# taiyaki-go/motioncheck_ccm_slam

Hardware: AMD Instinct MI355X
Metric: ORB extract+match Mfeatures/s and GBA iter/s (2k KF, 200k pts) @1/2/4/8 GPU (higher is better)
Workload: dtype u8; 1 GPU; configs[1]: 256 synthetic 752x480 frames per GPU, 8-level pyramid, 1000 features, FAST+quadtree+rBRIEF, then 1000x1000 brute-force Hamming on the 255 consecutive pairs; frames_per_gpu=256

## Files before the change

### include/ccm_hot.h

```cpp
#ifndef CCM_HOT_H
#define CCM_HOT_H

#include <stddef.h>
#include <stdint.h>

#ifdef __cplusplus
extern "C" {
#endif

#define CCM_ABI_VERSION 3

enum {
    CCM_OK = 0,
    CCM_E_ARG = -1,
    CCM_E_DEVICE = -2,
    CCM_E_NOMEM = -3,
    CCM_E_CAPACITY = -4,
    CCM_E_NUMERIC = -5,
    CCM_E_COMM = -6,
    CCM_E_STATE = -7
};

typedef struct ccm_ctx ccm_ctx;

// ... 16 lines not shown

typedef struct {
    int   nfeatures;
    float scale_factor;
    int   nlevels;
    int   ini_th_fast;
    int   min_th_fast;
} ccm_orb_params;

#define CCM_MAX_LEVELS 16

typedef struct {
    float x, y;
    float size;
    float angle;
    float response;
    int32_t octave;
    int32_t class_id;
} ccm_keypoint;

int ccm_orb_tables(const ccm_orb_params*, float* scale, float* inv_scale, float* sigma2,
                   float* inv_sigma2, int32_t* features_per_level, int32_t* umax);
int ccm_orb_level_sizes(const ccm_orb_params*, int w, int h, int32_t* level_w, int32_t* level_h);

int ccm_orb_extract(ccm_ctx*, const ccm_orb_params*, const uint8_t* img, int w, int h, int stride,
                    size_t image_stride, int n_images, ccm_keypoint* kps, uint8_t* desc,
                    int32_t* counts, int max_per_image);

int ccm_orb_extract_dev(ccm_ctx*, const ccm_orb_params*, const uint8_t* img_dev, int w, int h,
                        int stride, size_t image_stride, int n_images, int max_per_image);
int ccm_orb_fetch(ccm_ctx*, ccm_keypoint* kps, uint8_t* desc, int32_t* counts);
int ccm_orb_result_dev(ccm_ctx*, const uint8_t** desc_dev, const int32_t** counts_dev,
                       int* max_per_image);

int ccm_orb_debug_level(ccm_ctx*, int image, int level, uint8_t* out, int out_stride);
int ccm_orb_debug_candidates(ccm_ctx*, int image, int level, int32_t* xy, int32_t* score, int max);

int ccm_descriptor_distance(const uint8_t* a, const uint8_t* b);

int ccm_hamming_match(ccm_ctx*, const uint8_t* q, int nq, const uint8_t* t, int nt, int n_pairs,
                      const int32_t* nq_n, const int32_t* nt_n,
                      int32_t* best_idx, int32_t* best_dist, int32_t* second_dist);
int ccm_hamming_match_dev(ccm_ctx*, const uint8_t* q_dev, int nq, size_t q_pair_stride,
                          const uint8_t* t_dev, int nt, size_t t_pair_stride, int n_pairs,
                          const int32_t* nq_n_dev, const int32_t* nt_n_dev,
                          int32_t* best_idx_dev, int32_t* best_dist_dev, int32_t* second_dist_dev);
// ... 248 lines not shown
```

### motioncheck_ccm_slam_amd/_lib.py

```python
from __future__ import annotations

import ctypes as C
import os

import numpy as np

_HERE = os.path.dirname(os.path.abspath(__file__))
LIB_PATH = os.environ.get("CCM_HOT_LIB") or os.path.join(_HERE, "libccm_hot.so")

CCM_OK = 0
ERRORS = {-1: "CCM_E_ARG", -2: "CCM_E_DEVICE", -3: "CCM_E_NOMEM", -4: "CCM_E_CAPACITY",
          -5: "CCM_E_NUMERIC", -6: "CCM_E_COMM", -7: "CCM_E_STATE"}
COMM_ID_BYTES = 128

KP_DTYPE = np.dtype([("x", "f4"), ("y", "f4"), ("size", "f4"), ("angle", "f4"), ("response", "f4"),
                     ("octave", "i4"), ("class_id", "i4")])

SYMBOLS = [
    "ccm_abi_version", "ccm_create", "ccm_destroy", "ccm_last_error", "ccm_sync", "ccm_stream",
    "ccm_host_register", "ccm_host_unregister", "ccm_profile_enable", "ccm_profile_read",
    "ccm_orb_tables", "ccm_orb_level_sizes", "ccm_orb_extract", "ccm_orb_extract_dev", "ccm_orb_fetch",
    "ccm_orb_result_dev", "ccm_orb_debug_level", "ccm_orb_debug_candidates",
    "ccm_descriptor_distance", "ccm_hamming_match", "ccm_hamming_match_dev", "ccm_ratio_test", "ccm_match_bow",
    "ccm_window_candidates", "ccm_search_by_projection", "ccm_search_by_projection_frame", "ccm_search_for_initialization", "ccm_fuse_select", "ccm_fuse_select_batch", "ccm_search_by_sim3", "ccm_search_by_projection_sim3", "ccm_search_by_projection_sim3_batch",
    "ccm_search_for_triangulation", "ccm_voc_create", "ccm_voc_destroy", "ccm_voc_words", "ccm_voc_transform", "ccm_voc_transform_dev",
    "ccm_bow_vector", "ccm_bow_score_l1", "ccm_distinctive_descriptors", "ccm_optimize_sim3", "ccm_optimize_essential_graph", "ccm_correct_map_points",
    "ccm_ba_solve", "ccm_ba_landmark_cuts", "ccm_pose_optimize", "ccm_comm_unique_id", "ccm_comm_init", "ccm_comm_attach", "ccm_comm_destroy",
    "ccm_pose_from_mat4f", "ccm_pose_to_mat4f",
    "ccm_frame_create", "ccm_frame_from_extract", "ccm_frame_destroy", "ccm_frame_size", "ccm_frame_set_map_points",
    "ccm_frame_get_map_points", "ccm_frame_debug_grid", "ccm_frame_search_by_projection", "ccm_frame_search_by_projection_frame",
    "ccm_frame_pose_optimize",
    "ccm_sim3_ransac_iterations", "ccm_sim3_solver_create", "ccm_sim3_solver_destroy", "ccm_sim3_solver_count", "ccm_sim3_solver_iterate",
    "ccm_sim3_solver_find", "ccm_sim3_solver_estimate", "ccm_sim3_solver_state", "ccm_sim3_solver_hypotheses",
]


class CcmError(RuntimeError):
    def __init__(self, code, text=""):
        super().__init__("%s (%d): %s" % (ERRORS.get(code, "CCM_E_?"), code, text))
        self.code = code


class OrbParams(C.Structure):
    _fields_ = [("nfeatures", C.c_int), ("scale_factor", C.c_float), ("nlevels", C.c_int),
# ... 68 lines not shown
    if not os.path.exists(LIB_PATH):
        raise ImportError("%s not found: build it with `make -C motioncheck_ccm_slam_amd/csrc` "
                          "(or __graft_entry__.build()); there is no CPU fallback" % LIB_PATH)
    lib = C.CDLL(LIB_PATH)
    if lib.ccm_abi_version() != ABI_VERSION:
        raise ImportError("%s has ABI version %d, this package mirrors version %d of include/ccm_hot.h: rebuild it"
                          % (LIB_PATH, lib.ccm_abi_version(), ABI_VERSION))
    lib.ccm_create.restype = C.c_void_p
    lib.ccm_create.argtypes = [C.c_int, C.c_int]
    lib.ccm_destroy.argtypes = [C.c_void_p]
    lib.ccm_destroy.restype = None
    lib.ccm_last_error.restype = C.c_char_p
    lib.ccm_last_error.argtypes = [C.c_void_p]
    lib.ccm_sync.argtypes = [C.c_void_p]
    lib.ccm_stream.restype = C.c_void_p
    lib.ccm_stream.argtypes = [C.c_void_p]
    vp = C.c_void_p
    lib.ccm_host_register.argtypes = [vp, vp, C.c_size_t]
    lib.ccm_host_unregister.argtypes = [vp, vp]
    lib.ccm_profile_enable.argtypes = [vp, C.c_int]
    lib.ccm_profile_read.argtypes = [vp, vp, vp]
    lib.ccm_orb_tables.argtypes = [C.POINTER(OrbParams)] + [vp] * 6
    lib.ccm_orb_level_sizes.argtypes = [C.POINTER(OrbParams), C.c_int, C.c_int, vp, vp]
    lib.ccm_orb_extract.argtypes = [vp, C.POINTER(OrbParams), vp, C.c_int, C.c_int, C.c_int, C.c_size_t, C.c_int,
                                    vp, vp, vp, C.c_int]
    lib.ccm_orb_extract_dev.argtypes = [vp, C.POINTER(OrbParams), vp, C.c_int, C.c_int, C.c_int, C.c_size_t,
                                        C.c_int, C.c_int]
    lib.ccm_orb_fetch.argtypes = [vp, vp, vp, vp]
    lib.ccm_orb_result_dev.argtypes = [vp, C.POINTER(vp), C.POINTER(vp), C.POINTER(C.c_int)]
    lib.ccm_orb_debug_level.argtypes = [vp, C.c_int, C.c_int, vp, C.c_int]
    lib.ccm_orb_debug_candidates.argtypes = [vp, C.c_int, C.c_int, vp, vp, C.c_int]
    lib.ccm_descriptor_distance.argtypes = [vp, vp]
    lib.ccm_hamming_match.argtypes = [vp, vp, C.c_int, vp, C.c_int, C.c_int, vp, vp, vp, vp, vp]
    lib.ccm_hamming_match_dev.argtypes = [vp, vp, C.c_int, C.c_size_t, vp, C.c_int, C.c_size_t, C.c_int,
                                          vp, vp, vp, vp, vp]
    lib.ccm_ratio_test.argtypes = [C.c_int, C.c_int, C.c_float, C.c_int, C.c_int]
    lib.ccm_match_bow.argtypes = [vp, C.POINTER(BowOptions), vp, vp, vp, vp, C.c_int, vp, vp, vp, vp, C.c_int, vp]
    lib.ccm_window_candidates.argtypes = [vp, C.POINTER(FrameGrid), C.c_int, vp, vp, vp, vp, vp, vp, C.c_int, vp, vp, vp]
    lib.ccm_search_by_projection.argtypes = [vp, C.POINTER(FrameGrid), vp, C.c_int, vp, vp, vp, vp, vp, vp, vp, vp, C.c_float, C.c_float, vp]
    lib.ccm_search_by_projection_frame.argtypes = [vp, C.POINTER(FrameGrid), vp, vp, C.c_int, vp, vp, vp, vp, vp, vp, vp, vp, C.c_float, C.c_int, C.c_int, vp]
    lib.ccm_search_for_initialization.argtypes = [vp, C.c_int, vp, vp, vp, C.POINTER(FrameGrid), vp, vp, C.c_int, C.c_float, C.c_int, vp]
    lib.ccm_fuse_select.argtypes = [vp, C.POINTER(FrameGrid), vp, vp, C.c_int, vp, vp, vp, vp, vp, C.c_float, C.c_int, C.c_int, vp, vp]
    lib.ccm_fuse_select_batch.argtypes = [vp, C.c_int, vp, vp, vp, vp, vp, vp, vp, vp, vp, C.c_float, C.c_int, C.c_int, vp, vp]
    lib.ccm_search_by_sim3.argtypes = [vp, C.POINTER(FrameGrid), vp, C.POINTER(FrameGrid), vp] + [vp] * 10 + [C.c_float, vp]
    lib.ccm_search_by_projection_sim3.argtypes = [vp, C.POINTER(FrameGrid), vp, C.c_int] + [vp] * 7 + [C.c_float, vp]
    lib.ccm_search_by_projection_sim3_batch.argtypes = [vp, C.c_int, vp, vp, vp] + [vp] * 7 + [C.c_float, vp, vp]
# ... 111 lines not shown
```

### motioncheck_ccm_slam_amd/csrc/orb_host.cpp

```cpp
#include "ccm_internal.h"
#include "orb_types.h"
#include <cmath>
#include <cfloat>
#include <algorithm>

extern "C" hipError_t orb_upload_pattern();
size_t orb_octree_lds_bytes(int list_cap);
void orb_launch_resize(hipStream_t, const OrbGeom&, int level, int dw, int dh, int nframes);
void orb_launch_score(hipStream_t, const OrbGeom&, int ntiles, int nframes);
void orb_launch_nms(hipStream_t, const OrbGeom&, const OrbCell*, int ncells, int nframes, unsigned* slots, int* cell_count);
void orb_launch_fast_cells(hipStream_t, const OrbGeom&, const OrbCell*, const OrbBand*, int nbands, int nframes, size_t lds_bytes,
                           int surv_cap, unsigned* slots, int* cell_count);
size_t orb_fast_cells_lds(int pitch, int bh, int surv_cap);
void orb_launch_octree(hipStream_t, const OrbGeom&, const OrbCell*, int nlevels, int nframes, int list_cap,
                       const unsigned* slots, const int* cell_count, unsigned* keysA, unsigned* keysB,
                       unsigned* out, int* out_count, int* status);
void orb_launch_orient_desc(hipStream_t, const OrbGeom&, int out_per_frame, int nframes, const unsigned* sel,
                            const int* sel_count, ccm_keypoint* kps, uint8_t* desc, int* counts, int max_per_image,
                            int* status);

namespace {

inline int cv_round(float v) { return (int)lrintf(v); }
inline int cv_round(double v) { return (int)lrint(v); }

struct OrbTables {
    float scale[ORB_MAX_LEVELS], inv_scale[ORB_MAX_LEVELS], sigma2[ORB_MAX_LEVELS], inv_sigma2[ORB_MAX_LEVELS];
    int nfeat[ORB_MAX_LEVELS];
    int umax[16];
};

// ... 29 lines not shown
        t->umax[v] = v0;
        ++v0;
    }
    return CCM_OK;
}

void linear_tables(int ssize, int dsize, std::vector<int>& ofs, std::vector<short>& ab)
{
    ofs.resize(dsize); ab.resize(2 * (size_t)dsize);
    const double inv_scale = (double)dsize / ssize;
    const double scale = 1. / inv_scale;
    for (int d = 0; d < dsize; d++) {
        float fx = (float)((d + 0.5) * scale - 0.5);
        int sx = (int)std::floor(fx);
        fx -= sx;
        if (sx < 0) { sx = 0; fx = 0.f; }
        if (sx >= ssize - 1) { sx = ssize - 1; fx = 0.f; }
        ofs[d] = sx;
        ab[2 * d] = (short)cv_round((1.f - fx) * 2048.f);
        ab[2 * d + 1] = (short)cv_round(fx * 2048.f);
    }
}

}

struct OrbState {
    ccm_orb_params par{}; int w = 0, h = 0, nframes = 0, max_per_image = 0;
    bool valid = false, pattern_up = false;
    OrbTables tab{};
    OrbGeom geom{};
    std::vector<OrbCell> cells;
    std::vector<OrbBand> bands; size_t band_lds = 0; bool fused = true; int surv_cap = 1024; hipStream_t copy_stream = nullptr; hipEvent_t copy_done = nullptr;
    hipStream_t down_stream = nullptr; hipEvent_t chunk_done = nullptr;
    DevBuf geom_dev, cells_dev, tables_dev, bands_dev;
    DevBuf pyr, smap, slots, cell_count, keysA, keysB, sel, sel_count, status;
    DevBuf img0;
    DevBuf kps, desc, counts;
    size_t pyr_off[ORB_MAX_LEVELS]{}, smap_off[ORB_MAX_LEVELS]{};
    const uint8_t* last_img = nullptr; int last_stride = 0; size_t last_image_stride = 0;
    bool have_result = false;
};

void orb_state_free(OrbState* s)
{
    if (!s) return;
    if (s->copy_done) (void)hipEventDestroy(s->copy_done);
    if (s->chunk_done) (void)hipEventDestroy(s->chunk_done);
    delete s;
}

static inline size_t align_up(size_t v, size_t a) { return (v + a - 1) / a * a; }

static int orb_prepare(ccm_ctx* c, const ccm_orb_params* p, int w, int h, int nframes, int max_per_image)
{
    if (!c->orb) c->orb = new OrbState();
    OrbState& S = *c->orb;
    const bool same = S.valid && std::memcmp(&S.par, p, sizeof *p) == 0 && S.w == w && S.h == h &&
                      S.nframes == nframes && S.max_per_image == max_per_image;
    if (same) return CCM_OK;
    S.valid = false; S.have_result = false;
    int rc = make_tables(p, &S.tab);
    if (rc) return ccm_fail(c, rc, "bad ORB parameters");
    if (p->ini_th_fast < 0 || p->ini_th_fast > 255 || p->min_th_fast < 0 || p->min_th_fast > 255)
        return ccm_fail(c, CCM_E_ARG, "FAST thresholds must be in [0,255]");
    OrbGeom& G = S.geom;
    std::memset(&G, 0, sizeof G);
    G.nlevels = p->nlevels; G.ini_th = p->ini_th_fast; G.min_th = p->min_th_fast;
    for (int i = 0; i < 16; i++) G.umax[i] = S.tab.umax[i];
    S.cells.clear();
    std::vector<int> tab_i; std::vector<short> tab_s;
    struct TabOff { size_t xofs, yofs, xab, yab; } toff[ORB_MAX_LEVELS]{};
    size_t pyr_bytes = 0, smap_bytes = 0;
    int slot_acc = 0, key_acc = 0, out_acc = 0, tile_acc = 0, max_quota = 0;
    for (int l = 0; l < p->nlevels; l++) {
        OrbLevel& L = G.lv[l];
        L.w = cv_round((float)w * S.tab.inv_scale[l]);
        L.h = cv_round((float)h * S.tab.inv_scale[l]);
        if (L.w < 2 * ORB_EDGE + 8 || L.h < 2 * ORB_EDGE + 8 || L.w > 4096 + 2 * ORB_BORDER || L.h > 4096 + 2 * ORB_BORDER)
            return ccm_fail(c, CCM_E_ARG, "level %d is %dx%d: unsupported image size", l, L.w, L.h);
        L.scale = S.tab.scale[l];
        L.kp_size = (float)(int)(31 * S.tab.scale[l]);
        L.quota = S.tab.nfeat[l];
        max_quota = std::max(max_quota, L.quota);
        L.spitch = (int)align_up(L.w, 64);
        L.splane = (long long)L.spitch * L.h;
        S.smap_off[l] = smap_bytes; smap_bytes += align_up((size_t)L.splane * nframes, 256);
        if (l > 0) {
            L.pitch = (int)align_up(L.w, 64);
            L.plane = (long long)L.pitch * L.h;
            S.pyr_off[l] = pyr_bytes; pyr_bytes += align_up((size_t)L.plane * nframes, 256);
            std::vector<int> xo, yo; std::vector<short> xa, ya;
            linear_tables(G.lv[l - 1].w, L.w, xo, xa);
            linear_tables(G.lv[l - 1].h, L.h, yo, ya);
            toff[l].xofs = tab_i.size(); tab_i.insert(tab_i.end(), xo.begin(), xo.end());
            toff[l].yofs = tab_i.size(); tab_i.insert(tab_i.end(), yo.begin(), yo.end());
            toff[l].xab = tab_s.size(); tab_s.insert(tab_s.end(), xa.begin(), xa.end());
            toff[l].yab = tab_s.size(); tab_s.insert(tab_s.end(), ya.begin(), ya.end());
        }
        const int minBX = ORB_BORDER, minBY = ORB_BORDER, maxBX = L.w - ORB_EDGE + 3, maxBY = L.h - ORB_EDGE + 3;
        const float width = (float)(maxBX - minBX), height = (float)(maxBY - minBY);
        const int nCols = (int)(width / 30.f), nRows = (int)(height / 30.f);
        L.bw = maxBX - minBX; L.bh = maxBY - minBY;
        L.cell_first = (int)S.cells.size();
        int key_cap = 0;
        if (nCols >= 1 && nRows >= 1) {
            const int wCell = (int)std::ceil(width / nCols), hCell = (int)std::ceil(height / nRows);
            for (int i = 0; i < nRows; i++) {
                const float iniY = (float)(minBY + i * hCell);
                float maxY = iniY + hCell + 6;
                if (iniY >= maxBY - 3) continue;
                if (maxY > maxBY) maxY = (float)maxBY;
                for (int j = 0; j < nCols; j++) {
                    const float iniX = (float)(minBX + j * wCell);
                    float maxX = iniX + wCell + 6;
                    if (iniX >= maxBX - 6) continue;
                    if (maxX > maxBX) maxX = (float)maxBX;
                    OrbCell cell{};
                    cell.level = (short)l; cell.x0 = (short)iniX; cell.y0 = (short)iniY;
                    cell.cw = (short)((int)maxX - (int)iniX); cell.ch = (short)((int)maxY - (int)iniY);
                    if (cell.cw > 65 || cell.ch > 65)
                        return ccm_fail(c, CCM_E_ARG, "FAST cell %dx%d exceeds the kernel tile", cell.cw, cell.ch);
                    const int rw = std::max(cell.cw - 6, 0), rh = std::max(cell.ch - 6, 0);
                    cell.slot_cap = ((rw + 1) / 2) * ((rh + 1) / 2);
                    cell.slot_first = slot_acc;
                    slot_acc += cell.slot_cap; key_cap += cell.slot_cap;
                    S.cells.push_back(cell);
                }
            }
        }
        L.ncells = (int)S.cells.size() - L.cell_first;
        L.roots = (int)std::round((float)(maxBX - minBX) / (maxBY - minBY));
        if (L.roots < 1 || L.roots > ORB_MAX_ROOTS)
            return ccm_fail(c, CCM_E_ARG, "level %d aspect ratio gives %d quadtree roots (1..%d supported)", l, L.roots, ORB_MAX_ROOTS);
        L.hx = (float)(maxBX - minBX) / L.roots;
        L.key_first = key_acc; L.key_cap = std::max(key_cap, 1); key_acc += L.key_cap;
        L.out_cap = std::max(L.quota + 4, 4 * L.roots);
        L.out_first = out_acc; out_acc += L.out_cap;
        L.tiles_x = (L.w + 63) / 64; L.tiles_y = (L.h + 63) / 64;
        L.tile_first = tile_acc; tile_acc += L.tiles_x * L.tiles_y;
    }
    S.bands.clear(); S.band_lds = 0;
    static const bool want_fused = !(getenv("CCM_ORB_FUSED") && atoi(getenv("CCM_ORB_FUSED")) == 0);
    S.fused = want_fused;
    static const int pcap = getenv("CCM_FC_PCAP") ? std::min(atoi(getenv("CCM_FC_PCAP")), 256) : 144;
    static const int scap = getenv("CCM_FC_SURV") ? atoi(getenv("CCM_FC_SURV")) : 3072;
    S.surv_cap = scap;
    for (size_t a = 0; a < S.cells.size();) {
        size_t b = a;
        const OrbCell& c0 = S.cells[a];
        const int xa = (c0.x0 - 4) & ~3;
        int pitch = 0;
        while (b < S.cells.size() && S.cells[b].level == c0.level && S.cells[b].y0 == c0.y0) {
            const int p2 = (int)align_up((size_t)(S.cells[b].x0 + S.cells[b].cw + 4 - xa), 16);
            if (b > a && (p2 > pcap || b - a >= ORB_BAND_CELLS)) break;
            pitch = p2; b++;
        }
        OrbBand band{};
        band.cell_first = (int)a; band.ncells = (int)(b - a); band.level = c0.level; band.xa = (short)xa; band.y0 = (short)c0.y0;
        band.pitch = (short)pitch; band.bh = (short)c0.ch;
        {
            const OrbCell& cl = S.cells[b - 1];
            const int PW = pitch / 4, PQ = std::max(pitch / 16, 1);
// ... 21 lines not shown
    for (int l = 0; l < p->nlevels; l++) list_cap = std::max(list_cap, G.lv[l].out_cap);
    G.list_cap = (int)align_up(list_cap + 4, 16);
    if (orb_octree_lds_bytes(G.list_cap) > 150 * 1024)
        return ccm_fail(c, CCM_E_ARG, "nfeatures too large for the quadtree kernel's LDS (list cap %d)", G.list_cap);
    if (max_per_image < 1) return ccm_fail(c, CCM_E_ARG, "max_per_image must be positive");

    CCM_RESERVE(c, S.pyr, std::max<size_t>(pyr_bytes, 256));
    CCM_RESERVE(c, S.smap, smap_bytes);
    CCM_RESERVE(c, S.slots, (size_t)G.slots_per_frame * nframes * 4);
    CCM_RESERVE(c, S.cell_count, (size_t)std::max(G.ncells, 1) * nframes * 4);
    CCM_RESERVE(c, S.keysA, (size_t)G.keys_per_frame * nframes * 4);
    CCM_RESERVE(c, S.keysB, (size_t)G.keys_per_frame * nframes * 4);
    CCM_RESERVE(c, S.sel, (size_t)G.out_per_frame * nframes * 4);
    CCM_RESERVE(c, S.sel_count, (size_t)p->nlevels * nframes * 4);
    CCM_RESERVE(c, S.status, 256);
    CCM_RESERVE(c, S.kps, (size_t)nframes * max_per_image * sizeof(ccm_keypoint));
    CCM_RESERVE(c, S.desc, (size_t)nframes * max_per_image * 32);
    CCM_RESERVE(c, S.counts, (size_t)nframes * 4);
    const size_t tab_bytes = align_up(tab_i.size() * 4, 16) + tab_s.size() * 2;
    CCM_RESERVE(c, S.tables_dev, std::max<size_t>(tab_bytes, 16));
    CCM_RESERVE(c, S.cells_dev, std::max<size_t>(S.cells.size(), 1) * sizeof(OrbCell));
    CCM_RESERVE(c, S.bands_dev, std::max<size_t>(S.bands.size(), 1) * sizeof(OrbBand));
    CCM_RESERVE(c, S.geom_dev, sizeof(OrbGeom));
    char* tb = S.tables_dev.as<char>();
    const size_t s_base = align_up(tab_i.size() * 4, 16);
    for (int l = 0; l < p->nlevels; l++) {
        OrbLevel& L = G.lv[l];
        L.smap = S.smap.as<uint8_t>() + S.smap_off[l];
        if (l > 0) {
            L.img = S.pyr.as<uint8_t>() + S.pyr_off[l];
            L.xofs = reinterpret_cast<const int*>(tb) + toff[l].xofs;
            L.yofs = reinterpret_cast<const int*>(tb) + toff[l].yofs;
            L.xab = reinterpret_cast<const short*>(tb + s_base) + toff[l].xab;
            L.yab = reinterpret_cast<const short*>(tb + s_base) + toff[l].yab;
        }
    }
    if (!tab_i.empty()) CCM_HIP(c, hipMemcpyAsync(tb, tab_i.data(), tab_i.size() * 4, hipMemcpyHostToDevice, c->stream));
    if (!tab_s.empty()) CCM_HIP(c, hipMemcpyAsync(tb + s_base, tab_s.data(), tab_s.size() * 2, hipMemcpyHostToDevice, c->stream));
    if (!S.cells.empty())
        CCM_HIP(c, hipMemcpyAsync(S.cells_dev.p, S.cells.data(), S.cells.size() * sizeof(OrbCell), hipMemcpyHostToDevice, c->stream));
    for (OrbBand& b : S.bands) {
        const OrbLevel& L = G.lv[b.level];
        b.img = b.level > 0 ? L.img : nullptr; b.plane = L.plane; b.lpitch = L.pitch;
    }
    if (!S.bands.empty())
        CCM_HIP(c, hipMemcpyAsync(S.bands_dev.p, S.bands.data(), S.bands.size() * sizeof(OrbBand), hipMemcpyHostToDevice, c->stream));
    CCM_HIP(c, hipStreamSynchronize(c->stream));
    if (!S.pattern_up) { CCM_HIP(c, orb_upload_pattern()); S.pattern_up = true; }
    S.par = *p; S.w = w; S.h = h; S.nframes = nframes; S.max_per_image = max_per_image;
    S.valid = true;
    S.last_img = nullptr;
    return CCM_OK;
}

static int orb_run(ccm_ctx* c, const uint8_t* img_dev, int stride, size_t image_stride, int frame0 = 0, int nrun = -1)
{
    OrbState& S = *c->orb;
    OrbGeom& G = S.geom;
    G.lv[0].img = img_dev; G.lv[0].pitch = stride; G.lv[0].plane = (long long)image_stride;
    G.frame0 = frame0;
    if (nrun < 0) nrun = S.nframes - frame0;
    const OrbGeom& gd = G;
    const OrbCell* cd = S.cells_dev.as<OrbCell>();
    hipStream_t st = c->stream;
    if (frame0 == 0) CCM_HIP(c, hipMemsetAsync(S.status.p, 0, 4, st));
    for (int l = 1; l < G.nlevels; l++) { ProfScope ps(c, CCM_PROF_RESIZE); orb_launch_resize(st, gd, l, G.lv[l].w, G.lv[l].h, nrun); }
    if (S.fused && !S.bands.empty()) {
        ProfScope ps(c, CCM_PROF_FAST_SCORE);
        orb_launch_fast_cells(st, gd, cd, S.bands_dev.as<OrbBand>(), (int)S.bands.size(), nrun, S.band_lds, S.surv_cap, S.slots.as<unsigned>(), S.cell_count.as<int>());
    } else {
        { ProfScope ps(c, CCM_PROF_FAST_SCORE); orb_launch_score(st, gd, G.ntiles, nrun); }
        if (G.ncells > 0) { ProfScope ps(c, CCM_PROF_CELL_NMS); orb_launch_nms(st, gd, cd, G.ncells, nrun, S.slots.as<unsigned>(), S.cell_count.as<int>()); }
    }
    { ProfScope ps(c, CCM_PROF_OCTREE);
    orb_launch_octree(st, gd, cd, G.nlevels, nrun, G.list_cap, S.slots.as<unsigned>(), S.cell_count.as<int>(),
                      S.keysA.as<unsigned>(), S.keysB.as<unsigned>(), S.sel.as<unsigned>(), S.sel_count.as<int>(),
                      S.status.as<int>()); }
    { ProfScope ps(c, CCM_PROF_ORIENT_DESC);
    orb_launch_orient_desc(st, gd, G.out_per_frame, nrun, S.sel.as<unsigned>(), S.sel_count.as<int>(),
                           S.kps.as<ccm_keypoint>(), S.desc.as<uint8_t>(), S.counts.as<int>(), S.max_per_image,
                           S.status.as<int>()); }
    CCM_HIP(c, hipGetLastError());
    S.have_result = true;
    return CCM_OK;
}

static int orb_check_status(ccm_ctx* c)
{
    OrbState& S = *c->orb;
// ... 25 lines not shown
    if (rc) return rc;
    for (int i = 0; i < p->nlevels; i++) {
        if (scale) scale[i] = t.scale[i];
        if (inv_scale) inv_scale[i] = t.inv_scale[i];
        if (sigma2) sigma2[i] = t.sigma2[i];
        if (inv_sigma2) inv_sigma2[i] = t.inv_sigma2[i];
        if (features_per_level) features_per_level[i] = t.nfeat[i];
    }
    if (umax) for (int i = 0; i < 16; i++) umax[i] = t.umax[i];
    return CCM_OK;
}

int ccm_orb_level_sizes(const ccm_orb_params* p, int w, int h, int32_t* level_w, int32_t* level_h)
{
    OrbTables t;
    int rc = make_tables(p, &t);
    if (rc) return rc;
    if (!level_w || !level_h) return CCM_E_ARG;
    for (int l = 0; l < p->nlevels; l++) {
        level_w[l] = cv_round((float)w * t.inv_scale[l]);
        level_h[l] = cv_round((float)h * t.inv_scale[l]);
    }
    return CCM_OK;
}

int ccm_orb_extract_dev(ccm_ctx* c, const ccm_orb_params* p, const uint8_t* img_dev, int w, int h, int stride,
                        size_t image_stride, int n_images, int max_per_image)
{
    RoctxRange roctx_("ccm_orb_extract_dev");
    return ccm_guard(c, "ccm_orb_extract_dev", [&]() -> int {
        if (!c || !p) return CCM_E_ARG;
        if (n_images == 0 || w == 0 || h == 0) return CCM_OK;
        if (!img_dev || w < 0 || h < 0 || n_images < 0 || stride < w || (n_images > 1 && image_stride < (size_t)stride * h))
            return ccm_fail(c, CCM_E_ARG, "bad image arguments");
        CCM_HIP(c, hipSetDevice(c->device));
        int rc = orb_prepare(c, p, w, h, n_images, max_per_image);
        if (rc) return rc;
        return orb_run(c, img_dev, stride, image_stride);
    });
}

int ccm_orb_fetch(ccm_ctx* c, ccm_keypoint* kps, uint8_t* desc, int32_t* counts)
{
    RoctxRange roctx_("ccm_orb_fetch");
    if (!c || !c->orb || !c->orb->have_result) return c ? ccm_fail(c, CCM_E_STATE, "no extraction to fetch") : CCM_E_ARG;
    OrbState& S = *c->orb;
// ... 130 lines not shown
```

### motioncheck_ccm_slam_amd/csrc/orb_kernels.hip

```cpp
#include <hip/hip_runtime.h>
#include "orb_types.h"
#include "../../include/ccm_orb_pattern.h"
#include "../../include/ccm_sincos.h"
#include "../../include/ccm_hot.h"

#define WAVE 64

typedef unsigned short fc_us2 __attribute__((ext_vector_type(2)));
__device__ __forceinline__ fc_us2 fc_pk(unsigned x) { return __builtin_bit_cast(fc_us2, x); }
__device__ __forceinline__ unsigned fc_u(fc_us2 x) { return __builtin_bit_cast(unsigned, x); }

__device__ __forceinline__ int lane_id() { return threadIdx.x & 63; }
__device__ __forceinline__ unsigned long long lanemask_lt() { return (1ull << lane_id()) - 1ull; }

__device__ __forceinline__ void xcd_work_item(int on, int& x, int& y)
{
    x = (int)blockIdx.x; y = (int)blockIdx.y;
    if (!on) return;
    const unsigned gx = gridDim.x, total = gx * gridDim.y;
    const unsigned lin = blockIdx.y * gx + blockIdx.x;
    unsigned w;
    if (on == 1) {
        const unsigned xcd = lin & 7u, q = total >> 3, rem = total & 7u;
        w = xcd * q + (xcd < rem ? xcd : rem) + (lin >> 3);
// ... 26 lines not shown
{
#pragma unroll
    for (int d = 32; d >= 1; d >>= 1) v += __shfl_xor(v, d, 64);
    return v;
}
__device__ __forceinline__ void wave_sum2_dpp(int& x, int& y)
{
#define WS2_STEP(ctrl, rows) { const int tx = __builtin_amdgcn_update_dpp(0, x, ctrl, rows, 0xf, false); \
                               const int ty = __builtin_amdgcn_update_dpp(0, y, ctrl, rows, 0xf, false); x += tx; y += ty; }
    WS2_STEP(0xb1, 0xf)
    WS2_STEP(0x4e, 0xf)
    WS2_STEP(0x141, 0xf)
    WS2_STEP(0x140, 0xf)
    WS2_STEP(0x142, 0xa)
    WS2_STEP(0x143, 0xc)
#undef WS2_STEP
    x = __builtin_amdgcn_readlane(x, 63);
    y = __builtin_amdgcn_readlane(y, 63);
}

#ifndef RS_ROWS
#define RS_ROWS 8
#endif
__global__ __launch_bounds__(256) void k_pyr_resize(const OrbGeom g, int level)
{
    const OrbLevel& D = g.lv[level];
    const OrbLevel& S = g.lv[level - 1];
    const int lane = threadIdx.x & 63;
    const int x4 = (blockIdx.x * 64 + lane) * 4;
    const int yb = (blockIdx.y * 4 + __builtin_amdgcn_readfirstlane(threadIdx.x >> 6)) * RS_ROWS;
    const int f = blockIdx.z + g.frame0;
    if (yb >= D.h) return;
    const uint8_t* src = S.img + (long long)f * S.plane;
    uint8_t* dstp = const_cast<uint8_t*>(D.img) + (long long)f * D.plane;
    int yo; unsigned ybb;
    {
        const int y = min(yb + (lane & (RS_ROWS - 1)), D.h - 1);
        yo = D.yofs[y];
        __builtin_memcpy(&ybb, D.yab + 2 * y, 4);
    }
    const uint8_t* r0p[RS_ROWS]; const uint8_t* r1p[RS_ROWS]; unsigned b0[RS_ROWS], b1[RS_ROWS];
#pragma unroll
    for (int r = 0; r < RS_ROWS; r++) {
        const int sy0 = __builtin_amdgcn_readlane(yo, r);
        const unsigned bb = (unsigned)__builtin_amdgcn_readlane((int)ybb, r);
        r0p[r] = src + (long long)sy0 * S.pitch;
        r1p[r] = src + (long long)min(sy0 + 1, S.h - 1) * S.pitch;
        b0[r] = bb & 0xFFFFu; b1[r] = bb >> 16;
    }
    if (x4 >= D.w) return;
    {
        int sxs[4]; unsigned abw[4];
        if (x4 + 3 < D.w) {
            int4 so; uint4 ab;
            __builtin_memcpy(&so, D.xofs + x4, 16);
            __builtin_memcpy(&ab, D.xab + 2 * x4, 16);
            sxs[0] = so.x; sxs[1] = so.y; sxs[2] = so.z; sxs[3] = so.w;
            abw[0] = ab.x; abw[1] = ab.y; abw[2] = ab.z; abw[3] = ab.w;
        } else {
#pragma unroll
            for (int i = 0; i < 4; i++) {
                const int x = min(x4 + i, D.w - 1);
                sxs[i] = D.xofs[x];
                __builtin_memcpy(&abw[i], D.xab + 2 * x, 4);
            }
        }
        const int base = min(sxs[0], S.w - 8);
        const int ba = min(base & ~3, S.pitch - 12);
        if (S.w >= 8 && S.pitch >= 12 && sxs[3] - base <= 7) {
            uint2 q0[RS_ROWS], q1[RS_ROWS];
            const unsigned sh = (unsigned)(base - ba);
            const bool sh4 = sh > 3u;
#pragma unroll
            for (int r = 0; r < RS_ROWS; r++) {
                const unsigned* p0 = reinterpret_cast<const unsigned*>(r0p[r] + (unsigned)ba);
                const unsigned* p1 = reinterpret_cast<const unsigned*>(r1p[r] + (unsigned)ba);
                const unsigned d00 = p0[0], d01 = p0[1], d02 = p0[2], d10 = p1[0], d11 = p1[1], d12 = p1[2];
                const unsigned l0 = sh4 ? d01 : d00, m0 = sh4 ? d02 : d01, l1 = sh4 ? d11 : d10, m1 = sh4 ? d12 : d11;
                q0[r].x = __builtin_amdgcn_alignbyte(m0, l0, sh); q0[r].y = __builtin_amdgcn_alignbyte(d02, m0, sh);
                q1[r].x = __builtin_amdgcn_alignbyte(m1, l1, sh); q1[r].y = __builtin_amdgcn_alignbyte(d12, m1, sh);
            }
            unsigned sel[4];
#pragma unroll
            for (int i = 0; i < 4; i++) {
                const unsigned o = (unsigned)(sxs[i] - base);
                sel[i] = 0x0c000c00u + o + (min(o + 1u, 7u) << 16);
            }
#pragma unroll
            for (int r = 0; r < RS_ROWS; r++) {
                unsigned out = 0;
#pragma unroll
                for (int i = 0; i < 4; i++) {
                    const unsigned h0 = __builtin_amdgcn_udot2(fc_pk(__builtin_amdgcn_perm(q0[r].y, q0[r].x, sel[i])), fc_pk(abw[i]), 0u, false);
                    const unsigned h1 = __builtin_amdgcn_udot2(fc_pk(__builtin_amdgcn_perm(q1[r].y, q1[r].x, sel[i])), fc_pk(abw[i]), 0u, false);
                    const unsigned v = ((__umul24(b0[r], h0 >> 4) >> 16) + (__umul24(b1[r], h1 >> 4) >> 16) + 2u) >> 2;
                    out |= v << (8 * i);
                }
                if (yb + r < D.h) *reinterpret_cast<unsigned*>(dstp + (long long)(yb + r) * D.pitch + (unsigned)x4) = out;
            }
            return;
        }
    }
    for (int r = 0; r < RS_ROWS && yb + r < D.h; r++) {
        unsigned out = 0;
#pragma unroll
        for (int i = 0; i < 4; i++) {
            const int x = min(x4 + i, D.w - 1);
            const int sx0 = D.xofs[x];
            const int sx1 = min(sx0 + 1, S.w - 1);
            const int a0 = D.xab[2 * x], a1 = D.xab[2 * x + 1];
            const int h0 = r0p[r][sx0] * a0 + r0p[r][sx1] * a1;
            const int h1 = r1p[r][sx0] * a0 + r1p[r][sx1] * a1;
            const int v = ((((int)b0[r] * (h0 >> 4)) >> 16) + (((int)b1[r] * (h1 >> 4)) >> 16) + 2) >> 2;
            out |= (unsigned)(v & 255) << (8 * i);
        }
        *reinterpret_cast<unsigned*>(dstp + (long long)(yb + r) * D.pitch + (unsigned)x4) = out;
    }
}

__host__ __device__ inline int fast_score16(int v, const int* r)
{
    int d[16];
#pragma unroll
    for (int k = 0; k < 16; k++) d[k] = v - r[k];
    int lo3[16], hi3[16];
#pragma unroll
    for (int k = 0; k < 16; k++) {
        const int a = d[k], b = d[(k + 1) & 15], c = d[(k + 2) & 15];
        lo3[k] = min(a, min(b, c));
        hi3[k] = max(a, max(b, c));
    }
    int A = -256, B = 256;
#pragma unroll
    for (int k = 0; k < 16; k++) {
        A = max(A, min(lo3[k], min(lo3[(k + 3) & 15], lo3[(k + 6) & 15])));
        B = min(B, max(hi3[k], max(hi3[(k + 3) & 15], hi3[(k + 6) & 15])));
    }
    return max(A, -B) - 1;
}
// ... 1060 lines not shown
            }
        }
        if (lane < 4) *reinterpret_cast<unsigned long long*>(drow + 8 * lane) = mybits;
        if (lane == 0) {
            const OrbLevel& L = g.lv[level_c];
            ccm_keypoint kp;
            kp.x = (float)cx; kp.y = (float)cy;
            if (level_c != 0) { kp.x *= L.scale; kp.y *= L.scale; }
            kp.size = L.kp_size; kp.angle = angle; kp.response = (float)score_c;
            kp.octave = level_c; kp.class_id = -1;
            kps[(long long)f * max_per_image + row_c] = kp;
        }
        if (!more) break;
    }
}

extern "C" hipError_t orb_upload_pattern()
{
    return hipMemcpyToSymbol(HIP_SYMBOL(c_pattern), ccm_orb_pattern, 1024);
}

size_t orb_octree_lds_bytes(int list_cap) { return (size_t)list_cap * OCT_NODE_LDS + 64 + 4 * (size_t)OCT_LDS_KEYS + 8 * (size_t)list_cap; }

void orb_launch_resize(hipStream_t s, const OrbGeom& g_dev, int level, int dw, int dh, int nframes)
{
    dim3 grid((dw + 255) / 256, (dh + 4 * RS_ROWS - 1) / (4 * RS_ROWS), nframes);
    hipLaunchKernelGGL(k_pyr_resize, grid, dim3(256), 0, s, g_dev, level);
}
void orb_launch_score(hipStream_t s, const OrbGeom& g_dev, int ntiles, int nframes)
{
    hipLaunchKernelGGL(k_fast_score, dim3(ntiles, nframes), dim3(256), 0, s, g_dev);
}
void orb_launch_nms(hipStream_t s, const OrbGeom& g_dev, const OrbCell* cells, int ncells, int nframes,
                    unsigned* slots, int* cell_count)
{
    hipLaunchKernelGGL(k_cell_nms, dim3((ncells + 3) / 4, nframes), dim3(256), 0, s, g_dev, cells, slots, cell_count);
}
void orb_launch_fast_cells(hipStream_t s, const OrbGeom& g_dev, const OrbCell* cells, const OrbBand* bands, int nbands, int nframes,
                           size_t lds_bytes, int surv_cap, unsigned* slots, int* cell_count)
{
    static const bool packed = !(getenv("CCM_FC_PACKED") && atoi(getenv("CCM_FC_PACKED")) == 0);
    static const int abl = getenv("CCM_FC_ABL") ? atoi(getenv("CCM_FC_ABL")) : 0;
    static const int xcd_on = getenv("CCM_ORB_XCD_FC") ? atoi(getenv("CCM_ORB_XCD_FC")) : (getenv("CCM_ORB_XCD") ? atoi(getenv("CCM_ORB_XCD")) : 0);
    static const size_t lds_min = getenv("CCM_FC_LDS_MIN") ? (size_t)atol(getenv("CCM_FC_LDS_MIN")) : 0;
    if (lds_bytes < lds_min) lds_bytes = lds_min;
    (void)surv_cap;
    if (packed) hipLaunchKernelGGL(k_fast_cells<true>, dim3(nbands, nframes), dim3(FC_TPB), lds_bytes, s, g_dev, cells, bands, slots, cell_count, 0, abl, xcd_on);
    else hipLaunchKernelGGL(k_fast_cells<false>, dim3(nbands, nframes), dim3(FC_TPB), lds_bytes, s, g_dev, cells, bands, slots, cell_count, 0, abl, xcd_on);
}
size_t orb_fast_cells_lds(int pitch, int bh, int surv_cap) { return fc_lds_bytes(pitch, bh, surv_cap); }
// ... 22 lines not shown
```

### motioncheck_ccm_slam_amd/csrc/orb_types.h

```cpp
#pragma once
#include <cstdint>

#define ORB_MAX_LEVELS 16
#define ORB_EDGE 19
#define ORB_BORDER 16
#define ORB_HALF_PATCH 15
#define ORB_MAX_ROOTS 8
#define ORB_PATCH_R 21
#define ORB_PATCH_D 43
#define ORB_BLUR_D 37

struct OrbLevel {
    const uint8_t* img; long long plane; int pitch;
    int w, h;
    uint8_t* smap; long long splane; int spitch;
    const int* xofs; const short* xab; const int* yofs; const short* yab;
    int cell_first, ncells;
    int tile_first, tiles_x, tiles_y;
    int quota;
    int roots; float hx;
    int bw, bh;
    int key_first, key_cap;
    int out_first, out_cap;
    float scale;
// ... 1 lines not shown
};

struct OrbCell {
    short level, x0, y0, cw, ch, pad;
    int slot_first, slot_cap;
};

struct OrbBand {
    const uint8_t* img;
    long long plane;
    int lpitch, w, h;
    int level;
    int cell_first, ncells;
    short xa, y0, pitch, bh;
    short c_lo, c_hi, dw_lo, dw_hi;
    unsigned pw_inv, pq_inv;
    short clo[4], cwd[4];
    int slot_first[4], slot_cap[4];
    int pad_[4];
};
#define ORB_BAND_CELLS 4
static_assert(sizeof(OrbBand) == 128, "two s_load_dwordx16");

struct OrbGeom {
    int nlevels, ncells, ntiles;
    int frame0;
    int ini_th, min_th;
    int slots_per_frame;
    int keys_per_frame;
    int out_per_frame;
    int list_cap;
    int umax[16];
    OrbLevel lv[ORB_MAX_LEVELS];
};
static_assert(sizeof(OrbGeom) <= 3584, "OrbGeom is passed by value in the kernel arguments (4 KiB limit)");
```

Before: 282.4 Mfeatures/s.

## Fuse per-level pyramid resize launches into one strip-partitioned kernel

Replaces the seven separate per-level resize launches with a single kernel. Each block owns a horizontal strip of one frame and walks all pyramid levels in turn, using a block barrier between levels. Host-precomputed row ranges include the extra source rows needed to compute the next level's strip, so some rows are computed redundantly but no cross-block dependency remains. The kernel also absorbs the status memset. This removes launch and inter-kernel drain overhead and keeps strip data cache-resident, at the cost of duplicated boundary rows and less parallelism per launch.

```diff
diff --git a/include/ccm_hot.h b/include/ccm_hot.h
--- a/include/ccm_hot.h
+++ b/include/ccm_hot.h
@@ -62,6 +62,8 @@
 int ccm_orb_tables(const ccm_orb_params*, float* scale, float* inv_scale, float* sigma2,
                    float* inv_sigma2, int32_t* features_per_level, int32_t* umax);
 int ccm_orb_level_sizes(const ccm_orb_params*, int w, int h, int32_t* level_w, int32_t* level_h);
+int ccm_orb_debug_strips(const ccm_orb_params*, int w, int h, int n_images, int32_t* ranges, int ranges_cap, int32_t* yofs,
+                         int yofs_cap);
 
 int ccm_orb_extract(ccm_ctx*, const ccm_orb_params*, const uint8_t* img, int w, int h, int stride,
                     size_t image_stride, int n_images, ccm_keypoint* kps, uint8_t* desc,
diff --git a/motioncheck_ccm_slam_amd/_lib.py b/motioncheck_ccm_slam_amd/_lib.py
--- a/motioncheck_ccm_slam_amd/_lib.py
+++ b/motioncheck_ccm_slam_amd/_lib.py
@@ -19,7 +19,7 @@
 SYMBOLS = [
     "ccm_abi_version", "ccm_create", "ccm_destroy", "ccm_last_error", "ccm_sync", "ccm_stream",
     "ccm_host_register", "ccm_host_unregister", "ccm_profile_enable", "ccm_profile_read",
-    "ccm_orb_tables", "ccm_orb_level_sizes", "ccm_orb_extract", "ccm_orb_extract_dev", "ccm_orb_fetch",
+    "ccm_orb_tables", "ccm_orb_level_sizes", "ccm_orb_debug_strips", "ccm_orb_extract", "ccm_orb_extract_dev", "ccm_orb_fetch",
     "ccm_orb_result_dev", "ccm_orb_debug_level", "ccm_orb_debug_candidates",
     "ccm_descriptor_distance", "ccm_hamming_match", "ccm_hamming_match_dev", "ccm_ratio_test", "ccm_match_bow",
     "ccm_window_candidates", "ccm_search_by_projection", "ccm_search_by_projection_frame", "ccm_search_for_initialization", "ccm_fuse_select", "ccm_fuse_select_batch", "ccm_search_by_sim3", "ccm_search_by_projection_sim3", "ccm_search_by_projection_sim3_batch",
@@ -134,6 +134,7 @@
     lib.ccm_profile_read.argtypes = [vp, vp, vp]
     lib.ccm_orb_tables.argtypes = [C.POINTER(OrbParams)] + [vp] * 6
     lib.ccm_orb_level_sizes.argtypes = [C.POINTER(OrbParams), C.c_int, C.c_int, vp, vp]
+    lib.ccm_orb_debug_strips.argtypes = [C.POINTER(OrbParams), C.c_int, C.c_int, C.c_int, vp, C.c_int, vp, C.c_int]
     lib.ccm_orb_extract.argtypes = [vp, C.POINTER(OrbParams), vp, C.c_int, C.c_int, C.c_int, C.c_size_t, C.c_int,
                                     vp, vp, vp, C.c_int]
     lib.ccm_orb_extract_dev.argtypes = [vp, C.POINTER(OrbParams), vp, C.c_int, C.c_int, C.c_int, C.c_size_t,
diff --git a/motioncheck_ccm_slam_amd/csrc/orb_host.cpp b/motioncheck_ccm_slam_amd/csrc/orb_host.cpp
--- a/motioncheck_ccm_slam_amd/csrc/orb_host.cpp
+++ b/motioncheck_ccm_slam_amd/csrc/orb_host.cpp
@@ -6,7 +6,7 @@
 
 extern "C" hipError_t orb_upload_pattern();
 size_t orb_octree_lds_bytes(int list_cap);
-void orb_launch_resize(hipStream_t, const OrbGeom&, int level, int dw, int dh, int nframes);
+void orb_launch_pyramid(hipStream_t, const OrbGeom&, const OrbStripRows* rows, int strips, int threads, int nframes, int* status);
 void orb_launch_score(hipStream_t, const OrbGeom&, int ntiles, int nframes);
 void orb_launch_nms(hipStream_t, const OrbGeom&, const OrbCell*, int ncells, int nframes, unsigned* slots, int* cell_count);
 void orb_launch_fast_cells(hipStream_t, const OrbGeom&, const OrbCell*, const OrbBand*, int nbands, int nframes, size_t lds_bytes,
@@ -82,6 +82,32 @@
     }
 }
 
+struct StripRange { int own_lo, own_hi, cmp_lo, cmp_hi; };
+void orb_strip_ranges(const int* lh, const std::vector<int>* yofs, int nlevels, int K, std::vector<StripRange>& out)
+{
+    out.assign((size_t)K * nlevels, StripRange{});
+    for (int s = 0; s < K; s++)
+        for (int l = nlevels - 1; l >= 0; l--) {
+            StripRange& R = out[(size_t)s * nlevels + l];
+            R.own_lo = (int)((long long)lh[l] * s / K); R.own_hi = (int)((long long)lh[l] * (s + 1) / K);
+            R.cmp_lo = R.own_lo; R.cmp_hi = R.own_hi;
+            if (l + 1 == nlevels) continue;
+            const StripRange& N = out[(size_t)s * nlevels + l + 1];
+            if (N.cmp_lo >= N.cmp_hi) continue;
+            const int lo = yofs[l + 1][N.cmp_lo], hi = std::min(yofs[l + 1][N.cmp_hi - 1] + 1, lh[l] - 1) + 1;
+            if (R.own_lo >= R.own_hi) { R.cmp_lo = lo; R.cmp_hi = hi; }
+            else { R.cmp_lo = std::min(R.own_lo, lo); R.cmp_hi = std::max(R.own_hi, hi); }
+        }
+}
+
+int orb_strip_count(int nrun)
+{
+    static const int forced = getenv("CCM_PYR_STRIPS") ? atoi(getenv("CCM_PYR_STRIPS")) : 0;
+    int K = forced > 0 ? 1 : nrun >= 128 ? 8 : nrun >= 16 ? 16 : 32;
+    while (K < forced && K < ORB_MAX_STRIPS) K *= 2;
+    return K;
+}
+
 }
 
 struct OrbState {
@@ -92,7 +118,7 @@
     std::vector<OrbCell> cells;
     std::vector<OrbBand> bands; size_t band_lds = 0; bool fused = true; int surv_cap = 1024; hipStream_t copy_stream = nullptr; hipEvent_t copy_done = nullptr;
     hipStream_t down_stream = nullptr; hipEvent_t chunk_done = nullptr;
-    DevBuf geom_dev, cells_dev, tables_dev, bands_dev;
+    DevBuf geom_dev, cells_dev, tables_dev, bands_dev, strips_dev;
     DevBuf pyr, smap, slots, cell_count, keysA, keysB, sel, sel_count, status;
     DevBuf img0;
     DevBuf kps, desc, counts;
@@ -131,6 +157,7 @@
     std::vector<int> tab_i; std::vector<short> tab_s;
     struct TabOff { size_t xofs, yofs, xab, yab; } toff[ORB_MAX_LEVELS]{};
     size_t pyr_bytes = 0, smap_bytes = 0;
+    std::vector<int> yofs_l[ORB_MAX_LEVELS]; int lh[ORB_MAX_LEVELS];
     int slot_acc = 0, key_acc = 0, out_acc = 0, tile_acc = 0, max_quota = 0;
     for (int l = 0; l < p->nlevels; l++) {
         OrbLevel& L = G.lv[l];
@@ -152,6 +179,7 @@
             std::vector<int> xo, yo; std::vector<short> xa, ya;
             linear_tables(G.lv[l - 1].w, L.w, xo, xa);
             linear_tables(G.lv[l - 1].h, L.h, yo, ya);
+            yofs_l[l] = yo;
             toff[l].xofs = tab_i.size(); tab_i.insert(tab_i.end(), xo.begin(), xo.end());
             toff[l].yofs = tab_i.size(); tab_i.insert(tab_i.end(), yo.begin(), yo.end());
             toff[l].xab = tab_s.size(); tab_s.insert(tab_s.end(), xa.begin(), xa.end());
@@ -198,6 +226,13 @@
         L.out_first = out_acc; out_acc += L.out_cap;
         L.tiles_x = (L.w + 63) / 64; L.tiles_y = (L.h + 63) / 64;
         L.tile_first = tile_acc; tile_acc += L.tiles_x * L.tiles_y;
+        lh[l] = L.h;
+    }
+    std::vector<OrbStripRows> strip_rows;
+    for (int K = 1; K <= ORB_MAX_STRIPS; K *= 2) {
+        std::vector<StripRange> sr;
+        orb_strip_ranges(lh, yofs_l, p->nlevels, K, sr);
+        for (const StripRange& r : sr) strip_rows.push_back(OrbStripRows{(unsigned short)r.cmp_lo, (unsigned short)(r.cmp_hi - r.cmp_lo)});
     }
     S.bands.clear(); S.band_lds = 0;
     static const bool want_fused = !(getenv("CCM_ORB_FUSED") && atoi(getenv("CCM_ORB_FUSED")) == 0);
@@ -265,6 +300,8 @@
     CCM_RESERVE(c, S.cells_dev, std::max<size_t>(S.cells.size(), 1) * sizeof(OrbCell));
     CCM_RESERVE(c, S.bands_dev, std::max<size_t>(S.bands.size(), 1) * sizeof(OrbBand));
     CCM_RESERVE(c, S.geom_dev, sizeof(OrbGeom));
+    CCM_RESERVE(c, S.strips_dev, strip_rows.size() * sizeof(OrbStripRows));
+    CCM_HIP(c, hipMemcpyAsync(S.strips_dev.p, strip_rows.data(), strip_rows.size() * sizeof(OrbStripRows), hipMemcpyHostToDevice, c->stream));
     char* tb = S.tables_dev.as<char>();
     const size_t s_base = align_up(tab_i.size() * 4, 16);
     for (int l = 0; l < p->nlevels; l++) {
@@ -306,8 +343,14 @@
     const OrbGeom& gd = G;
     const OrbCell* cd = S.cells_dev.as<OrbCell>();
     hipStream_t st = c->stream;
-    if (frame0 == 0) CCM_HIP(c, hipMemsetAsync(S.status.p, 0, 4, st));
-    for (int l = 1; l < G.nlevels; l++) { ProfScope ps(c, CCM_PROF_RESIZE); orb_launch_resize(st, gd, l, G.lv[l].w, G.lv[l].h, nrun); }
+    if (G.nlevels == 1) { if (frame0 == 0) CCM_HIP(c, hipMemsetAsync(S.status.p, 0, 4, st)); }
+    else {
+        static const int threads = getenv("CCM_PYR_THREADS") ? atoi(getenv("CCM_PYR_THREADS")) : 256;
+        const int K = orb_strip_count(nrun);
+        const OrbStripRows* rows = S.strips_dev.as<OrbStripRows>() + (size_t)G.nlevels * (K - 1);
+        ProfScope ps(c, CCM_PROF_RESIZE);
+        orb_launch_pyramid(st, gd, rows, K, threads, nrun, frame0 == 0 ? S.status.as<int>() : nullptr);
+    }
     if (S.fused && !S.bands.empty()) {
         ProfScope ps(c, CCM_PROF_FAST_SCORE);
         orb_launch_fast_cells(st, gd, cd, S.bands_dev.as<OrbBand>(), (int)S.bands.size(), nrun, S.band_lds, S.surv_cap, S.slots.as<unsigned>(), S.cell_count.as<int>());
@@ -379,6 +422,28 @@
         level_h[l] = cv_round((float)h * t.inv_scale[l]);
     }
     return CCM_OK;
+}
+
+int ccm_orb_debug_strips(const ccm_orb_params* p, int w, int h, int n_images, int32_t* ranges, int ranges_cap, int32_t* yofs, int yofs_cap)
+{
+    OrbTables t;
+    int rc = make_tables(p, &t);
+    if (rc) return rc;
+    if (w < 1 || h < 1 || n_images < 1 || !ranges) return CCM_E_ARG;
+    int lh[ORB_MAX_LEVELS]; std::vector<int> yo[ORB_MAX_LEVELS]; std::vector<short> ab;
+    size_t ny = 0;
+    for (int l = 0; l < p->nlevels; l++) {
+        lh[l] = cv_round((float)h * t.inv_scale[l]);
+        if (lh[l] < 1) return CCM_E_ARG;
+        if (l > 0) { linear_tables(lh[l - 1], lh[l], yo[l], ab); ny += yo[l].size(); }
+    }
+    const int K = orb_strip_count(n_images);
+    if ((size_t)ranges_cap < (size_t)K * p->nlevels || (yofs && (size_t)yofs_cap < ny)) return CCM_E_ARG;
+    std::vector<StripRange> sr;
+    orb_strip_ranges(lh, yo, p->nlevels, K, sr);
+    std::memcpy(ranges, sr.data(), sr.size() * sizeof(StripRange));
+    if (yofs) for (int l = 1; l < p->nlevels; l++) yofs = std::copy(yo[l].begin(), yo[l].end(), yofs);
+    return K;
 }
 
 int ccm_orb_extract_dev(ccm_ctx* c, const ccm_orb_params* p, const uint8_t* img_dev, int w, int h, int stride,
diff --git a/motioncheck_ccm_slam_amd/csrc/orb_kernels.hip b/motioncheck_ccm_slam_amd/csrc/orb_kernels.hip
--- a/motioncheck_ccm_slam_amd/csrc/orb_kernels.hip
+++ b/motioncheck_ccm_slam_amd/csrc/orb_kernels.hip
@@ -72,24 +72,22 @@
 #ifndef RS_ROWS
 #define RS_ROWS 8
 #endif
-__global__ __launch_bounds__(256) void k_pyr_resize(const OrbGeom g, int level)
+typedef __attribute__((address_space(1))) const uint8_t pyr_gu8;
+typedef __attribute__((address_space(1))) const unsigned pyr_gu32;
+typedef __attribute__((address_space(1))) unsigned pyr_gu32w;
+__device__ __forceinline__ void pyr_item(const OrbGeom& g, int level, int f, int yb, int y_end, int x4)
 {
     const OrbLevel& D = g.lv[level];
     const OrbLevel& S = g.lv[level - 1];
-    const int lane = threadIdx.x & 63;
-    const int x4 = (blockIdx.x * 64 + lane) * 4;
-    const int yb = (blockIdx.y * 4 + __builtin_amdgcn_readfirstlane(threadIdx.x >> 6)) * RS_ROWS;
-    const int f = blockIdx.z + g.frame0;
-    if (yb >= D.h) return;
-    const uint8_t* src = S.img + (long long)f * S.plane;
-    uint8_t* dstp = const_cast<uint8_t*>(D.img) + (long long)f * D.plane;
+    pyr_gu8* src = (pyr_gu8*)S.img + (long long)f * S.plane;
+    pyr_gu8* dstp = (pyr_gu8*)D.img + (long long)f * D.plane;
     int yo; unsigned ybb;
     {
-        const int y = min(yb + (lane & (RS_ROWS - 1)), D.h - 1);
+        const int y = min(yb + ((x4 >> 2) & (RS_ROWS - 1)), y_end - 1);
         yo = D.yofs[y];
         __builtin_memcpy(&ybb, D.yab + 2 * y, 4);
     }
-    const uint8_t* r0p[RS_ROWS]; const uint8_t* r1p[RS_ROWS]; unsigned b0[RS_ROWS], b1[RS_ROWS];
+    pyr_gu8* r0p[RS_ROWS]; pyr_gu8* r1p[RS_ROWS]; unsigned b0[RS_ROWS], b1[RS_ROWS];
 #pragma unroll
     for (int r = 0; r < RS_ROWS; r++) {
         const int sy0 = __builtin_amdgcn_readlane(yo, r);
@@ -123,8 +121,8 @@
             const bool sh4 = sh > 3u;
 #pragma unroll
             for (int r = 0; r < RS_ROWS; r++) {
-                const unsigned* p0 = reinterpret_cast<const unsigned*>(r0p[r] + (unsigned)ba);
-                const unsigned* p1 = reinterpret_cast<const unsigned*>(r1p[r] + (unsigned)ba);
+                pyr_gu32* p0 = (pyr_gu32*)(r0p[r] + (unsigned)ba);
+                pyr_gu32* p1 = (pyr_gu32*)(r1p[r] + (unsigned)ba);
                 const unsigned d00 = p0[0], d01 = p0[1], d02 = p0[2], d10 = p1[0], d11 = p1[1], d12 = p1[2];
                 const unsigned l0 = sh4 ? d01 : d00, m0 = sh4 ? d02 : d01, l1 = sh4 ? d11 : d10, m1 = sh4 ? d12 : d11;
                 q0[r].x = __builtin_amdgcn_alignbyte(m0, l0, sh); q0[r].y = __builtin_amdgcn_alignbyte(d02, m0, sh);
@@ -146,12 +144,17 @@
                     const unsigned v = ((__umul24(b0[r], h0 >> 4) >> 16) + (__umul24(b1[r], h1 >> 4) >> 16) + 2u) >> 2;
                     out |= v << (8 * i);
                 }
-                if (yb + r < D.h) *reinterpret_cast<unsigned*>(dstp + (long long)(yb + r) * D.pitch + (unsigned)x4) = out;
+                *(pyr_gu32w*)(dstp + (long long)min(yb + r, y_end - 1) * D.pitch + (unsigned)x4) = out;
             }
             return;
         }
     }
-    for (int r = 0; r < RS_ROWS && yb + r < D.h; r++) {
+#pragma unroll 1
+    for (int y = yb; y < min(yb + RS_ROWS, y_end); y++) {
+        const int sy0 = D.yofs[y];
+        pyr_gu8* r0 = src + (long long)sy0 * S.pitch;
+        pyr_gu8* r1 = src + (long long)min(sy0 + 1, S.h - 1) * S.pitch;
+        const int w0 = D.yab[2 * y], w1 = D.yab[2 * y + 1];
         unsigned out = 0;
 #pragma unroll
         for (int i = 0; i < 4; i++) {
@@ -159,12 +162,36 @@
             const int sx0 = D.xofs[x];
             const int sx1 = min(sx0 + 1, S.w - 1);
             const int a0 = D.xab[2 * x], a1 = D.xab[2 * x + 1];
-            const int h0 = r0p[r][sx0] * a0 + r0p[r][sx1] * a1;
-            const int h1 = r1p[r][sx0] * a0 + r1p[r][sx1] * a1;
-            const int v = ((((int)b0[r] * (h0 >> 4)) >> 16) + (((int)b1[r] * (h1 >> 4)) >> 16) + 2) >> 2;
+            const int h0 = r0[sx0] * a0 + r0[sx1] * a1;
+            const int h1 = r1[sx0] * a0 + r1[sx1] * a1;
+            const int v = (((w0 * (h0 >> 4)) >> 16) + ((w1 * (h1 >> 4)) >> 16) + 2) >> 2;
             out |= (unsigned)(v & 255) << (8 * i);
         }
-        *reinterpret_cast<unsigned*>(dstp + (long long)(yb + r) * D.pitch + (unsigned)x4) = out;
+        *(pyr_gu32w*)(dstp + (long long)y * D.pitch + (unsigned)x4) = out;
+    }
+}
+
+template <int T>
+__global__ __launch_bounds__(T) void k_pyr_strips(const OrbGeom g, const OrbStripRows* __restrict__ rows, int* status)
+{
+    const int f = blockIdx.y + g.frame0;
+    const int wave = __builtin_amdgcn_readfirstlane(threadIdx.x >> 6);
+    if (status && blockIdx.x == 0 && blockIdx.y == 0 && threadIdx.x == 0) *status = 0;
+    rows += blockIdx.x * g.nlevels;
+    for (int l = 1; l < g.nlevels; l++) {
+        const int lo = rows[l].lo, y_end = lo + rows[l].n;
+        const int xg = (g.lv[l].w + 255) >> 8;
+        int yb = lo, xq = wave;
+        while (xq >= xg) { xq -= xg; yb += RS_ROWS; }
+        while (yb < y_end) {
+            int lane;
+            asm volatile("v_mbcnt_lo_u32_b32 %0, -1, 0\n\tv_mbcnt_hi_u32_b32 %0, -1, %0" : "=v"(lane));
+            pyr_item(g, l, f, yb, y_end, (xq * 64 + lane) * 4);
+            xq += T / 64;
+            while (xq >= xg) { xq -= xg; yb += RS_ROWS; }
+        }
+        __threadfence_block();
+        __syncthreads();
     }
 }
 
@@ -1271,10 +1298,12 @@
 
 size_t orb_octree_lds_bytes(int list_cap) { return (size_t)list_cap * OCT_NODE_LDS + 64 + 4 * (size_t)OCT_LDS_KEYS + 8 * (size_t)list_cap; }
 
-void orb_launch_resize(hipStream_t s, const OrbGeom& g_dev, int level, int dw, int dh, int nframes)
-{
-    dim3 grid((dw + 255) / 256, (dh + 4 * RS_ROWS - 1) / (4 * RS_ROWS), nframes);
-    hipLaunchKernelGGL(k_pyr_resize, grid, dim3(256), 0, s, g_dev, level);
+void orb_launch_pyramid(hipStream_t s, const OrbGeom& g_dev, const OrbStripRows* rows, int strips, int threads, int nframes, int* status)
+{
+    dim3 grid(strips, nframes);
+    if (threads == 1024) hipLaunchKernelGGL(k_pyr_strips<1024>, grid, dim3(1024), 0, s, g_dev, rows, status);
+    else if (threads == 512) hipLaunchKernelGGL(k_pyr_strips<512>, grid, dim3(512), 0, s, g_dev, rows, status);
+    else hipLaunchKernelGGL(k_pyr_strips<256>, grid, dim3(256), 0, s, g_dev, rows, status);
 }
 void orb_launch_score(hipStream_t s, const OrbGeom& g_dev, int ntiles, int nframes)
 {
diff --git a/motioncheck_ccm_slam_amd/csrc/orb_types.h b/motioncheck_ccm_slam_amd/csrc/orb_types.h
--- a/motioncheck_ccm_slam_amd/csrc/orb_types.h
+++ b/motioncheck_ccm_slam_amd/csrc/orb_types.h
@@ -47,6 +47,9 @@
 #define ORB_BAND_CELLS 4
 static_assert(sizeof(OrbBand) == 128, "two s_load_dwordx16");
 
+struct alignas(4) OrbStripRows { unsigned short lo, n; };
+#define ORB_MAX_STRIPS 64
+
 struct OrbGeom {
     int nlevels, ncells, ntiles;
     int frame0;
```

Measured after the change: 267.4 Mfeatures/s. 5.3% lower.
